# leonsick/depthg

Measured on AMD Instinct MI355X. Metric: correlation-loss steps/sec at B=32,C=384,28x28 (fwd+bwd, per-GPU batch 32), higher is better.
Workload: dtype bf16 (feats) / f16 (code) MFMA inputs, f32 accumulate

## Files before the change

depthg_amd/csrc/dg_api_corr.hip:

```cpp
#include "dg_api.h"
#include "dg_corr_args.h"
#include "dg_taps.h"

static unsigned long long* g_prof_span = nullptr;
extern "C" int dg_prof_main_span(void* span) { g_prof_span = static_cast<unsigned long long*>(span); return DG_OK; }

enum class Prep { Small, Dense, General };
enum class Sampler { Plane, ChannelLast };
enum class MainKernel { Small, Corr2, CorrMain };
enum class Depth { None, Job, GsBlocks, GsOwnLaunch };
enum class Hist { Rows, Blobs };
enum class Masks { None, Sampled, DenseRaw, DenseSplit };

struct PairSet {
    int op;
    int neg;
    bool mapped;
    float shift;
    int slot_loss, slot_cd;
    float fin_scale;
    int gidx, csel, dest;
    float factor;
};
struct Operand {
    int srcsel;
    int cset;
    int map;
};

struct Plan {
    int B, C, D, h, w, hc, wc, S, Sh, P, Ppad, KF, KD, C4, D4, N, T, nops, rf, nrb;
    bool shared, depth, grad, pointwise;
    Prep prep;
    Sampler sampler;
    MainKernel main;
    Masks masks;
    Hist hist;
    bool fold;
    bool half;
    Depth depth_run;
    int nsplit;
    int dep_nrb;
    float lo, hi;
    float shift_depth;
    float inv_numel;
    float grad_f, grad_fn;
    int blob, blob_off_c;
    PairSet ps[DG_MAX_NEG + 2];
    Operand ops[DG_MAX_NEG + 2];
    bool gr_on;
    int gr_nkeys, gr_cpb, gr_blocks_per_image;
    int8_t gr_key[DG_MAX_JOBS], gr_first[DG_MAX_JOBS];
    int32_t gr_nblk[DG_MAX_JOBS];
    size_t nhwc_f[2], nhwc_c[2];
    size_t rows_f[DG_MAX_NEG + 2], rows_c[DG_MAX_NEG + 2];
    size_t op[DG_MAX_NEG + 2], inv[DG_MAX_NEG + 2], colpart[DG_MAX_NEG + 2], bbar[DG_MAX_NEG + 2];
    size_t ccolpart[DG_MAX_NEG + 2], csum[DG_MAX_NEG + 2], bsplit[DG_MAX_NEG + 2];
    size_t rvec[DG_MAX_NEG + 2], rimg[DG_MAX_NEG + 2];
    size_t nz, nzsum;
    size_t dRA[DG_MAX_NEG + 3], dRB[DG_MAX_NEG + 2];
    size_t part[DG_MAX_NEG + 3];
    size_t comb[2], scratch_out, taps, gbuf[DG_MAX_NEG + 2];
    size_t ticket;
    size_t maskbits[DG_MAX_NEG + 2];
    size_t clo[2];
    size_t gr_list, gr_count, gr_rank;
    size_t dRA2[DG_MAX_NEG + 2], dRBs[DG_MAX_NEG + 2], dRB2[DG_MAX_NEG + 2][2], dRBm[DG_MAX_NEG + 2], part4, om;
    size_t total;

    bool small() const { return prep == Prep::Small; }
    bool dense() const { return prep == Prep::Dense; }
    bool plane() const { return sampler == Sampler::Plane; }
    bool has_masks() const { return masks != Masks::None; }
    bool depth_in_gs() const { return depth_run == Depth::GsBlocks || depth_run == Depth::GsOwnLaunch; }
    bool dense_masks() const { return masks == Masks::DenseRaw || masks == Masks::DenseSplit; }
    bool intra_symmetric() const { return !pointwise || fold; }
    const int64_t* batch_map(int k, const int64_t* perms) const {
        return k < 0 ? nullptr : reinterpret_cast<const int64_t*>(reinterpret_cast<uintptr_t>(perms) + (size_t)k * B * sizeof(int64_t));
    }
    const int64_t* map_of(int t, const int64_t* perms) const { return batch_map(ps[t].mapped ? ps[t].neg : -1, perms); }
};

static inline float* f32(char* ws, size_t off) { return reinterpret_cast<float*>(ws + off); }

#define FOLD_STASH_OFF (5 * 1024)

static void plan_tables(const dg_corr_desc* d, Plan& p) {
    const double numel = (double)p.B * p.P * p.P;
    p.inv_numel = (float)(1.0 / numel);
    p.grad_f = (float)(-1.0 / numel);
    p.grad_fn = p.N > 0 ? p.grad_f / (float)p.N : 0.f;
    for (int t = 0; t < p.T; ++t) {
        PairSet& s = p.ps[t];
        const bool neg = t >= 2;
        s.neg = neg ? t - 2 : -1;
        s.mapped = neg && p.shared;
        s.op = s.mapped ? 0 : t;
        s.shift = t == 0 ? d->shift_intra : (t == 1 ? d->shift_inter : d->shift_neg);
        s.slot_loss = neg ? DG_OUT_LOSS_NEG : t;
        s.slot_cd = neg ? DG_OUT_CD_NEG : DG_OUT_CD_INTRA + t;
        s.fin_scale = neg ? (float)(1.0 / (numel * p.N)) : p.inv_numel;
        s.gidx = neg ? 2 : t; s.csel = t == 0 ? 0 : 1; s.dest = t == 1 ? 1 : 0;
        s.factor = neg ? p.grad_fn : p.grad_f;
    }
    for (int o = 0; o < p.nops; ++o) p.ops[o] = Operand{o == 1 ? 1 : 0, o == 0 ? 0 : 1, o >= 2 ? o - 2 : -1};
    const int L = (p.Ppad / 32) % 8;
    if (!(p.grad && p.KF == 384 && p.KD == 96 && p.D <= 80 && p.nrb > 1 && L >= 1 && L <= 4 && p.B % 8 == 0 && p.B <= 64)) return;
    int nkeys = 0, members[DG_MAX_JOBS] = {0};
    for (int t = 0; t < p.T; ++t) {
        int k = -1;
        for (int q = 0; q < nkeys; ++q) if (p.ps[p.gr_first[q]].op == p.ps[t].op) k = q;
        if (k < 0) { k = nkeys++; p.gr_first[k] = (int8_t)t; }
        p.gr_key[t] = (int8_t)k; ++members[k];
    }
    for (int k = 0; k < nkeys; ++k) p.gr_on |= members[k] > 1;
    if (!p.gr_on) return;
    p.gr_nkeys = nkeys; p.gr_cpb = 8 / L;
// ... 66 lines not shown
    for (int i = 0; i < p.nops; ++i) { p.rows_f[i] = take(want_rows ? B * p.P * frow : 0); p.rows_c[i] = take(want_rows ? B * p.P * p.D4 * 4 : 0); }
    for (int i = 0; i < p.nops; ++i) {
        p.op[i] = take(B * (p.Ppad / 32) * (size_t)p.blob);
        p.inv[i] = take(B * p.Ppad * 4);
        p.colpart[i] = take(B * (size_t)(ident ? p.h * ((p.w + 31) / 32) : p.Ppad / 32) * p.KF * 4);
        p.bbar[i] = take(B * p.KF * 4);
        p.bsplit[i] = take(B * 2 * p.KF * 2);
        p.ccolpart[i] = take(B * (size_t)(p.Ppad / 32) * p.KD * 4);
        p.csum[i] = take(B * p.KD * 4);
    }
    for (int t = 0; t < p.T; ++t) { p.rvec[t] = take(B * p.Ppad * 4); p.rimg[t] = take(B * 4); }
    p.nz = take(B * p.Ppad * 4);
    p.nzsum = take(B * 4);
    for (int t = 0; t <= p.T; ++t) { p.dRA[t] = take(B * p.Ppad * p.KD * 4); p.part[t] = take(B * p.nrb * 2 * 4); }
    for (int t = 0; t < p.T; ++t) p.dRB[t] = take(B * p.Ppad * p.KD * 4);
    for (int i = 0; i < 2; ++i) p.comb[i] = take(B * p.Ppad * p.KD * 4);
    p.scratch_out = take(DG_OUT_COUNT * 4);
    p.taps = take(2 * B * dg_taps_record_bytes(p.hc * p.wc, p.P));
    for (int t = 0; t < p.T; ++t) p.gbuf[t] = p.grad ? take(B * (size_t)(p.Ppad / 32) * (p.Ppad / 32) * 2048) : 0;
    p.ticket = take(256);
    const bool xmask = rows && !p.small() && p.grad && plain_zero_clamp && p.Ppad <= 256 && p.rf == 4;
    const bool xmask_dense = (d->flags & DG_EXACT_MASKS) && ident && p.grad && plain_zero_clamp &&
                             p.KF == 384 && p.KD == 96 && p.D <= 80 && p.Ppad >= 160 && p.B <= 64;
    if ((d->flags & DG_EXACT_MASKS) && p.grad && (d->flags & DG_ZERO_CLAMP) && !xmask && !xmask_dense && !p.small())
        return fail(DG_ERR_UNSUPPORTED, "DG_EXACT_MASKS: exact clamp masks exist on small sample grids (always on there) and on the dense "
                                        "identity grid with C <= 384 (padded to 384), D <= 80, P >= 160, B <= 64, zero_clamp without stabalize");
    p.masks = xmask ? Masks::Sampled : (!xmask_dense ? Masks::None : (p.pointwise ? Masks::DenseSplit : Masks::DenseRaw));
    for (int t = 0; t < p.T; ++t) p.maskbits[t] = take(p.has_masks() ? B * (size_t)(p.Ppad / 32) * p.Ppad * 4 : 0);
    p.main = p.small() ? MainKernel::Small
                       : (p.grad && dg_corr2_shape_supported(p.KF, p.KD, p.D, p.lo, p.hi, p.Ppad, p.B) ? MainKernel::Corr2 : MainKernel::CorrMain);
    static const bool fold_on = [] { const char* e = getenv("DG_FOLD_INTRA"); return !(e && e[0] == '0'); }();
    p.fold = fold_on && p.main == MainKernel::Corr2 && p.pointwise && !xmask;
    p.half = p.main == MainKernel::Corr2 && ident && p.N * p.B <= 512 && p.S == p.h && p.S == p.w;
    p.depth_run = (!p.depth || p.small()) ? Depth::None : (!p.grad ? Depth::Job : (p.dense_masks() ? Depth::GsOwnLaunch : Depth::GsBlocks));
    for (int i = 0; i < 2; ++i) p.clo[i] = take(p.masks == Masks::DenseSplit ? B * (size_t)(p.Ppad / 32) * p.KD * 64 : 0);
    p.gr_list = take((size_t)DG_MAX_JOBS * B * DG_GR_CAP * 4);
    p.gr_count = take((size_t)DG_MAX_JOBS * B * 4);
    p.gr_rank = take((size_t)DG_MAX_JOBS * B * 2);
    {
        const bool sg = p.small() && p.grad, two = sg && p.pointwise;
        const size_t gt = B * p.Ppad * p.KD * 4;
        for (int t = 0; t < p.T; ++t) {
            p.dRA2[t] = take(two ? gt : 0);
            p.dRBs[t] = take(sg && p.nsplit == 2 ? gt : 0);
            for (int k = 0; k < 2; ++k) p.dRB2[t][k] = take(two && k < p.nsplit ? gt : 0);
            p.dRBm[t] = take(sg && t >= 2 && (p.pointwise || p.nsplit == 2) ? gt : 0);
        }
        p.part4 = take(p.small() ? (size_t)(p.T + 1) * B * p.nsplit * 16 : 0);
        p.om = take(p.small() ? (size_t)(p.T + 1) * 4 : 0);
    }
    p.total = off;
    plan_tables(d, p);
    return DG_OK;
}

extern "C" size_t dg_corr_workspace_bytes(const dg_corr_desc* desc) {
    Plan p{};
    if (make_plan(desc, p) != DG_OK) return 0;
    return p.total;
}

static DgJob helper_job(const Plan& p, char* ws, int t, bool passB, const int64_t* perms) {
    DgJob j;
    memset(&j, 0, sizeof(j));
    const int o2 = p.ps[t].op;
    const int64_t* m2 = p.map_of(t, perms);
// ... 312 lines not shown
    DgColmeanArgs m;
    memset(&m, 0, sizeof(m));
    m.nops = p.nops; m.B = p.B; m.P = p.P; m.Ppad = p.Ppad; m.KF = p.KF; m.KD = p.KD;
    for (int o = 0; o < p.nops; ++o) {
        m.colpart[o] = p.pointwise ? f32(c.ws, p.colpart[o]) : nullptr; m.bbar[o] = f32(c.ws, p.bbar[o]);
        m.bsplit[o] = reinterpret_cast<__bf16*>(c.ws + p.bsplit[o]);
        m.ngroups[o] = p.Ppad / 32;
        m.ccolpart[o] = f32(c.ws, p.ccolpart[o]); m.csum[o] = f32(c.ws, p.csum[o]);
    }
    m.zero_word = p.depth_in_gs() ? reinterpret_cast<unsigned int*>(c.ws + p.ticket) : nullptr;
    m.zero_words9 = a.wctr;
    if (p.gr_on) {
        m.gr.nh = p.T; m.gr.nkeys = p.gr_nkeys; m.gr.B = p.B;
        for (int t = 0; t < p.T; ++t) { m.gr.sidx[t] = p.map_of(t, c.perms); m.gr.key[t] = p.gr_key[t]; }
        m.gr.list = reinterpret_cast<int32_t*>(c.ws + p.gr_list); m.gr.count = reinterpret_cast<int32_t*>(c.ws + p.gr_count);
        m.gr.rank = reinterpret_cast<int16_t*>(c.ws + p.gr_rank);
    }
    if (p.dense() && p.pointwise) {
        m.dc.code[0] = c.code; m.dc.code[1] = c.code_pos;
        for (int o = 0; o < 2; ++o) { m.dc.blob[o] = c.ws + p.op[o]; m.dc.inv_norm[o] = f32(c.ws, p.inv[o]); m.dc.ccolpart[o] = f32(c.ws, p.ccolpart[o]); }
        m.dc.B = p.B; m.dc.D = p.D; m.dc.KF = p.KF; m.dc.KD = p.KD; m.dc.h = p.h; m.dc.w = p.w; m.dc.P = p.P; m.dc.Ppad = p.Ppad;
        if (p.masks == Masks::DenseSplit) { m.dc.clo[0] = c.ws + p.clo[0]; m.dc.clo[1] = c.ws + p.clo[1]; }
    }
    if (c.split) {
        DgColmeanArgs ms = m;
        ms.zsel = 1; m.zsel = 2;
        DG_HIP(c.side->hand_over(0));
        DG_HIP(dg_launch_colmean(ms, c.side->stream()));
    }
    DG_HIP(dg_launch_colmean(m, c.stream));
    return DG_OK;
}

static int fwd_cd_mask3(Fwd& c) {
    const Plan& p = c.p;
    DgCdMask3Args m;
    memset(&m, 0, sizeof(m));
    m.opR = c.ws + p.op[0]; m.loR = c.ws + p.clo[0];
    for (int t = 0; t < p.T; ++t) {
        m.opS[t] = c.ws + p.op[p.ps[t].op]; m.loS[t] = c.ws + p.clo[p.ps[t].op]; m.sidx[t] = p.map_of(t, c.perms);
        m.bits[t] = reinterpret_cast<uint32_t*>(c.ws + p.maskbits[t]);
    }
    m.T = p.T; m.B = p.B; m.Ppad = p.Ppad; m.blob_bytes = p.blob; m.off_c = p.blob_off_c; m.KD = p.KD;
    if (c.split) {
        DG_HIP(c.side->hand_over(1));
        DG_HIP(dg_launch_cd_mask3(m, c.side->stream()));
        DG_HIP(c.side->record_join());
    } else {
        DG_HIP(dg_launch_cd_mask3(m, c.stream));
    }
    return DG_OK;
}

static int fwd_rowmeans(Fwd& c) {
    const Plan& p = c.p;
    DgRowmeanArgs r;
    memset(&r, 0, sizeof(r));
    r.B = p.B; r.P = p.P; r.Ppad = p.Ppad; r.KF = p.KF; r.KD = p.KD; r.njobs = p.T; r.abar = f32(c.ws, p.bbar[0]);
    for (int t = 0; t < p.T; ++t) {
        r.jobs[t].A = c.ws + p.op[0]; r.jobs[t].aidx = nullptr;
        r.jobs[t].bbar = f32(c.ws, p.bbar[p.ps[t].op]); r.jobs[t].bidx = p.map_of(t, c.perms);
        r.jobs[t].bsplit = reinterpret_cast<const __bf16*>(c.ws + p.bsplit[p.ps[t].op]);
        r.jobs[t].rvec = f32(c.ws, p.rvec[t]); r.jobs[t].rimg = f32(c.ws, p.rimg[t]);
    }
    if (p.dense()) {
        r.ncs = 2;
// ... 51 lines not shown
        DG_HIP(side.fork());
        DG_HIP(dg_launch_gs(g, dep_maskbits, side.stream(), true));
        DG_HIP(side.record_join());
        DG_HIP(dg_launch_gs(gstream, nullptr, c.stream, false, p.half));
        DG_HIP(side.join());
    } else {
        DG_HIP(dg_launch_gs(gstream, nullptr, c.stream, false, p.half));
        DG_HIP(dg_launch_gs(g, dep_maskbits, c.stream, true));
    }
    return DG_OK;
}

static int corr_forward_impl(const dg_corr_desc* desc, const float* orig_feats, const float* orig_feats_pos,
                             const float* orig_code, const float* orig_code_pos, const float* depth,
                             const float* coords1, const float* coords2, const int64_t* perms, const DrawArgs* draw,
                             float* out_scalars, void* workspace, size_t workspace_bytes, dg_stream_t stream_,
                             const FeatKeep* fk = nullptr, const float* feat_inv = nullptr) {
    Fwd c;
    if (int rc = make_plan(desc, c.p)) return rc;
    const Plan& p = c.p;
    c.desc = desc; c.feats = orig_feats; c.feats_pos = orig_feats_pos; c.code = orig_code; c.code_pos = orig_code_pos; c.depth = depth;
    c.coords1 = coords1; c.coords2 = coords2; c.perms = perms; c.draw = draw; c.fk = fk; c.feat_inv = feat_inv; c.out = out_scalars;
    c.stream = static_cast<hipStream_t>(stream_);
    if (int rc = fwd_validate(c, workspace, workspace_bytes)) return rc;

    if (p.dense_masks() && split_masks_enabled()) c.side.emplace(c.stream);
    c.split = c.side && static_cast<bool>(*c.side) && p.pointwise;

    if (p.small()) return forward_small(c);
    if (int rc = p.dense() ? fwd_operands_dense(c) : fwd_operands_general(c)) return rc;

    build_corr_jobs(p, c.ws, perms, c.a);

    if (int rc = fwd_colmeans(c)) return rc;
    if (p.masks == Masks::DenseSplit) { if (int rc = fwd_cd_mask3(c)) return rc; }
    if (p.pointwise) { if (int rc = fwd_rowmeans(c)) return rc; }

    if (c.split) DG_HIP(c.side->join());
    if (int rc = launch_main(p, c.a, c.stream)) return rc;

    return fwd_finish(c);
}

extern "C" int dg_corr_forward(const dg_corr_desc* desc, const float* orig_feats, const float* orig_feats_pos,
                               const float* orig_code, const float* orig_code_pos, const float* depth,
                               const float* coords1, const float* coords2, const int64_t* perms,
                               float* out_scalars, void* workspace, size_t workspace_bytes, dg_stream_t stream_) {
    return corr_forward_impl(desc, orig_feats, orig_feats_pos, orig_code, orig_code_pos, depth, coords1, coords2, perms, nullptr,
                             out_scalars, workspace, workspace_bytes, stream_);
}

extern "C" int dg_corr_forward_extnorm(const dg_corr_desc* desc, const float* orig_feats, const float* orig_feats_pos,
                                       const float* orig_code, const float* orig_code_pos, const float* depth,
                                       const float* coords1, const float* coords2, const int64_t* perms, const float* feat_inv,
                                       float* out_scalars, void* workspace, size_t workspace_bytes, dg_stream_t stream_) {
    if (!feat_inv) return fail(DG_ERR_INVALID, "dg_corr_forward_extnorm: feat_inv is null");
    return corr_forward_impl(desc, orig_feats, orig_feats_pos, orig_code, orig_code_pos, depth, coords1, coords2, perms, nullptr,
                             out_scalars, workspace, workspace_bytes, stream_, nullptr, feat_inv);
}

extern "C" int dg_sampled_sumsq(int32_t B, int32_t C, int32_t h, int32_t w, int32_t S, int32_t line_grid, const float* feats,
                                const float* coords, const int64_t* srcidx, int32_t accumulate, float* out, dg_stream_t stream_) {
    if (B < 1 || C < 1 || h < 1 || w < 1 || S < 1 || !feats || !coords || !out) return fail(DG_ERR_INVALID, "dg_sampled_sumsq: bad arguments");
    DG_HIP(dg_launch_sampled_sumsq(feats, coords, srcidx, out, B, C, h, w, S, line_grid ? 1 : S, accumulate ? 1 : 0, static_cast<hipStream_t>(stream_)));
    return DG_OK;
}

extern "C" int dg_corr_forward_draw(const dg_corr_desc* desc, const float* orig_feats, const float* orig_feats_pos,
                                    const float* orig_code, const float* orig_code_pos, const float* depth,
// ... 238 lines not shown
```

depthg_amd/csrc/dg_corr_args.h:

```cpp
#pragma once
#include "dg_device.h"

__host__ __device__ inline int dg_perm32(int pl) {
    int s = pl >> 4, u = (pl >> 3) & 1, hh = (pl >> 2) & 1, v = pl & 3;
    return (2 * s + hh) * 8 + 4 * u + v;
}

#ifndef DG_F_IG
#define DG_F_IG 4
#endif
__host__ __device__ inline int dg_f_off(int q, int g) {
    constexpr int IG = DG_F_IG;
    return ((g / IG) * 32 + q) * (IG * 16) + (((g % IG) ^ ((q / (16 / IG)) % IG)) * 16);
}

struct DgBlob {
    int GF, GD, KD;
    int off_c, off_p, bytes;
    __host__ __device__ DgBlob(int KF, int KD_) : GF(KF / 8), GD(KD_ / 8), KD(KD_) {
        off_c = 32 * GF * 16;
        off_p = off_c + GD * 32 * 16;
        bytes = off_p + 4 * KD * 16;
    }
    __host__ __device__ int f(int q, int g) const { return dg_f_off(q, g); }
// ... 338 lines not shown
struct DgColmeanArgs {
    const float* colpart[DG_MAX_NEG + 2];
    float* bbar[DG_MAX_NEG + 2];
    __bf16* bsplit[DG_MAX_NEG + 2];
    const float* ccolpart[DG_MAX_NEG + 2];
    float* csum[DG_MAX_NEG + 2];
    int32_t ngroups[DG_MAX_NEG + 2];
    int32_t nops, B, P, Ppad, KF, KD;
    unsigned int* zero_word;
    unsigned int* zero_words9;
    DgGroupArgs gr;
    DgDenseCodeArgs dc;
    int32_t zsel;
};

struct DgRowmeanJob {
    const char* A;
    const float* bbar;
    const __bf16* bsplit;
    const int64_t* aidx;
    const int64_t* bidx;
    float* rvec;
    float* rimg;
};
struct DgRowmeanArgs {
    DgRowmeanJob jobs[DG_MAX_NEG + 2];
    int32_t njobs, B, P, Ppad, KF, KD;
    const float* abar;
    char* stash;
    int32_t stash_off;
    const float* cs_part[2];
    float* cs_out[2];
    int32_t ncs;
};

struct DgScatterSrc {
    const float* buf;
    const int64_t* route;
    int32_t gidx;
    int32_t coords_sel;
    float factor;
    int32_t dest;
    int32_t raw;
    const float* dfac;
    int32_t half;
};
#define DG_MAX_SCATTER 48
struct DgScatterArgs {
    DgScatterSrc src[DG_MAX_SCATTER];
    int32_t nsrc;
    const float* coords1;
    const float* coords2;
    const float* gscal;
    const float* gtot;
    float wtot[4];
    float* comb[2];
    char* taps;
    const char* xop;
    const float* xinv;
    const float* xinv_dest[2];
    int32_t blob_bytes, blob_off_c;
    float* out[2];
    int32_t B, D, DP, h, w, S, Sh, P, Ppad, DC;
    int32_t dense;
    int8_t craw[2][DG_MAX_SCATTER / 2], cfin[2][DG_MAX_SCATTER / 2];
    int8_t ncraw[2], ncfin[2];
// ... 45 lines not shown
hipError_t dg_launch_gs(const struct DgGsArgs& a, const uint32_t* dep_maskbits, hipStream_t s, bool depth_only = false, bool half_out = false);
hipError_t dg_launch_finish(const DgFinishArgs& a, hipStream_t stream);
hipError_t dg_launch_transpose(const DgTransposeArgs& a, int B, hipStream_t s);
hipError_t dg_launch_gather(const DgGatherArgs& a, int maxK, hipStream_t s);
hipError_t dg_launch_cd_mask(const DgCdMaskArgs& a, hipStream_t s);
struct DgCdMask3Args {
    const char* opR;
    const char* loR;
    const char* opS[DG_MAX_NEG + 2];
    const char* loS[DG_MAX_NEG + 2];
    const int64_t* sidx[DG_MAX_NEG + 2];
    uint32_t* bits[DG_MAX_NEG + 2];
    int32_t T, B, Ppad, blob_bytes, off_c, KD;
    int32_t nsplit;
};
hipError_t dg_launch_cd_mask3(const DgCdMask3Args& a, hipStream_t s);
#define DG_HIST_MAX_BINS 256
struct DgCdHistArgs {
    const char* opR;
    const char* opS[DG_MAX_NEG + 2];
    const float* rowsR;
    const float* rowsS[DG_MAX_NEG + 2];
    const int64_t* sidx[DG_MAX_NEG + 2];
    unsigned long long* out;
    int32_t count, B, P, Ppad, D, D4, KD, blob_bytes, off_c;
    int32_t nbins;
    float lo, scale;
};
hipError_t dg_launch_cd_hist(const DgCdHistArgs& a, bool rows, hipStream_t s);
hipError_t dg_launch_plane_sample(const DgPlaneArgs& a, hipStream_t s);
hipError_t dg_launch_colmean(const DgColmeanArgs& a, hipStream_t s);
hipError_t dg_launch_prep_dense(const DgDenseArgs& a, hipStream_t s);
hipError_t dg_launch_rowmean(const DgRowmeanArgs& a, hipStream_t s);
hipError_t dg_launch_set_stash(char* blobs, int B, int ntiles, size_t blob_bytes, int off, const float* rvec, int P, int Ppad, hipStream_t s);
hipError_t dg_launch_scatter(const DgScatterArgs& a, hipStream_t s);
hipError_t dg_launch_super_perms(const float* keys, uint64_t seed, unsigned long long* state, int count, int B, int64_t* out, hipStream_t s);
hipError_t dg_launch_pre_general(const struct DgPreArgs& a, hipStream_t s);
bool dg_small_supported(int Ppad, int KD);
hipError_t dg_launch_corr_small(const struct DgSmallArgs& a, hipStream_t s);
hipError_t dg_launch_small_finish(const struct DgSmallArgs& a, hipStream_t s);
hipError_t dg_launch_gather_rows(const struct DgGatherRowsArgs& a, hipStream_t s);
hipError_t dg_launch_rand_coords_state(unsigned long long* state, float* out, int n, hipStream_t s, float keep_p = -1.f);
hipError_t dg_launch_fps(const float* depth, const float* depth_b, int Ba, int B, int H, int W, int h, int w, int S, float factor,
                         float* out_coords, int32_t* out_inds, float* pooled_ws, hipStream_t s);
hipError_t dg_launch_sampled_sumsq(const float* feats, const float* coords, const int64_t* srcidx, float* out, int B, int C, int h, int w, int S, int Sh, int accumulate, hipStream_t s);
hipError_t dg_launch_normalize_split(const float* src, int B, int C, int P, int nchunks, int chunk_c, float* const* dst, hipStream_t s);
```

depthg_amd/csrc/dg_prep.hip:

```cpp
#include "dg_device.h"
#include "dg_corr_args.h"
#include "dg_taps.h"
#include <cstdlib>

__global__ void k_nchw_to_nhwc(const DgTransposeArgs a) {
    __shared__ float t[32][33];
    const int b = blockIdx.z;
    int m = 0, gy = blockIdx.y;
    while (m < a.nmaps - 1 && gy >= (a.K4[m] + 31) / 32) { gy -= (a.K4[m] + 31) / 32; ++m; }
    const float* __restrict__ src = a.src[m];
    float* __restrict__ dst = a.dst[m];
    const int K = a.K[m], K4 = a.K4[m], HW = a.HW[m];
    const int k0 = gy * 32, p0 = blockIdx.x * 32;
    if (p0 >= HW) return;
    const int tx = threadIdx.x, ty = threadIdx.y;
    for (int i = ty; i < 32; i += 8) {
        int k = k0 + i, p = p0 + tx;
        t[i][tx] = (k < K && p < HW) ? src[((size_t)b * K + k) * HW + p] : 0.f;
    }
    __syncthreads();
    for (int i = ty; i < 32; i += 8) {
        int p = p0 + i, k = k0 + tx;
        if (p < HW && k < K4) dst[((size_t)b * HW + p) * K4 + k] = t[tx][i];
    }
// ... 664 lines not shown
            v[e] = *reinterpret_cast<const _Float16*>(xt + (tl * 32 + pl) * RS + d * 2);
        }
        *reinterpret_cast<f16x8*>(blob0 + (size_t)tl * L.bytes + L.p(d, cc)) = v;
    }
    for (int id = tid; id < ntile * KD; id += 256) {
        const int tl = id / KD, d = id - tl * KD;
        float cs = 0.f;
#pragma unroll 8
        for (int qq = 0; qq < 32; ++qq) cs += (float)*reinterpret_cast<const _Float16*>(xt + (tl * 32 + qq) * RS + d * 2);
        a.ccolpart[o][((size_t)n * nt + t0 + tl) * KD + d] = cs;
    }
}

template <int UN>
__device__ __forceinline__ void prep_dense_code_norms(const DgDenseArgs& a, int xb, int n, int o) {
    const int HW = a.h * a.w, i = xb * 256 + threadIdx.x;
    float* inv = a.inv_norm[o] + (size_t)n * a.Ppad;
    if (xb == 0)
        for (int p = a.P + threadIdx.x; p < a.Ppad; p += 256) inv[p] = 0.f;
    if (i >= HW) return;
    const float* src = a.code[o] + (size_t)n * a.D * HW + i;
    float t[4 * UN];
#pragma unroll
    for (int k = 0; k < 4 * UN; ++k) t[k] = k < a.D ? src[(size_t)k * HW] : 0.f;
    float ss[4] = {0.f, 0.f, 0.f, 0.f};
#pragma unroll
    for (int u = 0; u < UN; ++u)
#pragma unroll
        for (int kg = 0; kg < 4; ++kg) ss[kg] = fmaf(t[kg + 4 * u], t[kg + 4 * u], ss[kg]);
    const float tot = ss[0] + ss[1] + ss[2] + ss[3];
    inv[i] = 1.f / fmaxf(sqrtf(tot), DG_EPS_NORM);
}

__device__ __forceinline__ void dense_code_planes(const DgDenseCodeArgs& a, char* xt, int n, int o, int g) {
    const int tid = threadIdx.x, HW = a.h * a.w, nt = a.Ppad / 32, KD = a.KD;
    const DgBlob L(a.KF, a.KD);
    const int nch = min(8, a.D - 8 * g);
    char* const xl = xt + (size_t)a.Ppad * 16;
    const bool want_lo = a.clo[o] != nullptr;
    for (int p = a.P + tid; p < a.Ppad; p += 256) {
        reinterpret_cast<uint4*>(xt)[p] = make_uint4(0u, 0u, 0u, 0u);
        if (want_lo) reinterpret_cast<uint4*>(xl)[p] = make_uint4(0u, 0u, 0u, 0u);
    }
    if (nch <= 0) {
        for (int p = tid; p < a.P; p += 256) {
            reinterpret_cast<uint4*>(xt)[p] = make_uint4(0u, 0u, 0u, 0u);
            if (want_lo) reinterpret_cast<uint4*>(xl)[p] = make_uint4(0u, 0u, 0u, 0u);
        }
    } else {
        const float* src = a.code[o] + ((size_t)n * a.D + 8 * g) * HW;
        const float* inv = a.inv_norm[o] + (size_t)n * a.Ppad;
        for (int i0 = 0; i0 < HW; i0 += 1024) {
            float t[4][8], iv[4];
            int pp[4];
#pragma unroll
            for (int j = 0; j < 4; ++j) {
                const int i = i0 + tid + 256 * j;
                const bool ok = i < HW;
                pp[j] = ok ? i : -1;
                iv[j] = ok ? inv[pp[j]] : 0.f;
#pragma unroll
                for (int c = 0; c < 8; ++c) t[j][c] = (ok && c < nch) ? src[(size_t)c * HW + i] : 0.f;
            }
#pragma unroll
            for (int j = 0; j < 4; ++j) {
                if (pp[j] < 0) continue;
                f16x8 v;
#pragma unroll
                for (int c = 0; c < 8; ++c) v[c] = c < nch ? (_Float16)(t[j][c] * iv[j]) : (_Float16)0.f;
                *reinterpret_cast<f16x8*>(xt + pp[j] * 16) = v;
                if (want_lo) {
                    f16x8 l;
#pragma unroll
                    for (int c = 0; c < 8; ++c) l[c] = c < nch ? (_Float16)((t[j][c] * iv[j] - (float)v[c]) * 2048.f) : (_Float16)0.f;
                    *reinterpret_cast<f16x8*>(xl + pp[j] * 16) = l;
                }
            }
        }
    }
    __syncthreads();
    char* blob0 = a.blob[o] + (size_t)n * nt * L.bytes;
    for (int id = tid; id < nt * 32; id += 256) {
        const int tl = id >> 5, qq = id & 31;
        *reinterpret_cast<uint4*>(blob0 + (size_t)tl * L.bytes + L.c(qq, g)) = reinterpret_cast<const uint4*>(xt)[id];
        if (want_lo)
            *reinterpret_cast<uint4*>(a.clo[o] + ((size_t)n * nt + tl) * (KD * 64) + (g * 32 + qq) * 16) = reinterpret_cast<const uint4*>(xl)[id];
    }
    for (int id = tid; id < nt * 32; id += 256) {
        const int tl = id >> 5, cc = (id >> 3) & 3, c = id & 7;
        f16x8 v;
#pragma unroll
        for (int e = 0; e < 8; ++e) {
            const int pl = 16 * (cc >> 1) + 8 * ((e >> 2) & 1) + 4 * (cc & 1) + (e & 3);
            v[e] = *reinterpret_cast<const _Float16*>(xt + (tl * 32 + pl) * 16 + c * 2);
        }
        *reinterpret_cast<f16x8*>(blob0 + (size_t)tl * L.bytes + L.p(8 * g + c, cc)) = v;
    }
    for (int id = tid; id < nt * 8; id += 256) {
        const int tl = id >> 3, c = id & 7;
        float cs = 0.f;
#pragma unroll 8
        for (int qq = 0; qq < 32; ++qq) cs += (float)*reinterpret_cast<const _Float16*>(xt + (tl * 32 + qq) * 16 + c * 2);
        a.ccolpart[o][((size_t)n * nt + tl) * KD + 8 * g + c] = cs;
    }
}


template <int MAXU, int UNC, bool FK = false>
__global__ __launch_bounds__(256) void k_prep_dense(const DgDenseArgs a) {
    extern __shared__ float sl[];
    int bid;
    {
        const int nwg = gridDim.x, orig = blockIdx.x;
        const int q = nwg >> 3, rem = nwg & 7, xcd = orig & 7;
        bid = (xcd < rem ? xcd * (q + 1) : rem * (q + 1) + (xcd - rem) * q) + (orig >> 3);
    }
    const int gx = a.Ppad / 32;
    const int nz = a.depth ? 5 : 4;
    const int x = bid % gx, z = (bid / gx) % nz, n = bid / (gx * nz);
    const int roles = a.roles ? a.roles : 15;
    if (n >= a.B) {
        if (roles & 8) dg_super_perm_row(nullptr, a.draw_seed, a.draw_state, a.B, a.draw_out, bid - gx * nz * a.B, a.draw_count, sl);
        return;
    }
    if (!(roles & (z < 2 ? 1 : (z < 4 ? 2 : 4)))) return;
    if (z < 2) {
        prep_dense_feats<MAXU, FK>(a, sl, x, n, z);
    } else if (z < 4) {
        if (a.code_split) {
            if (x * 256 < a.h * a.w) prep_dense_code_norms<UNC>(a, x, n, z - 2);
        } else if (x * DENSE_TPB < a.Ppad / 32) prep_dense_code<UNC>(a, sl, x, n, z - 2);
    } else if (x == 0) {
        depth_nz_image(a.depth, a.nz, a.nzsum, n, a.dH, a.dW, a.h, a.h, a.Ppad, true);
    }
}

// ... 96 lines not shown
__device__ __forceinline__ void colsum_reduce(const float* part, int n, int ngroups, int K, float scale, float* out) {
    for (int k = threadIdx.x; k < K; k += blockDim.x) {
        const float* cp = part + (size_t)n * ngroups * K + k;
        float s = 0.f;
        int t = 0;
        for (; t + 16 <= ngroups; t += 16) {
            float v[16];
#pragma unroll
            for (int u = 0; u < 16; ++u) v[u] = cp[(size_t)(t + u) * K];
#pragma unroll
            for (int u = 0; u < 16; ++u) s += v[u];
        }
        for (; t + 4 <= ngroups; t += 4) {
            float v[4];
#pragma unroll
            for (int u = 0; u < 4; ++u) v[u] = cp[(size_t)(t + u) * K];
#pragma unroll
            for (int u = 0; u < 4; ++u) s += v[u];
        }
        for (; t < ngroups; ++t) s += cp[(size_t)t * K];
        out[(size_t)n * K + k] = s * scale;
    }
}

__global__ __launch_bounds__(256) void k_colmean(const DgColmeanArgs a) {
    extern __shared__ __attribute__((aligned(16))) char cm_smem[];
    const int n = blockIdx.x, o = blockIdx.y;
    if (a.zero_word && n == 0 && o == 0 && blockIdx.z == 0 && threadIdx.x == 0) *a.zero_word = 0u;
    if (a.zero_words9 && n == 0 && o == 0 && blockIdx.z == 0 && threadIdx.x < 9) a.zero_words9[threadIdx.x] = 0u;
    auto reduce = [&](const float* part, int ngroups, int K, float scale, float* out) __attribute__((always_inline)) { colsum_reduce(part, n, ngroups, K, scale, out); };
    if (a.zsel == 1 ? blockIdx.z != 3 : (a.zsel == 2 && blockIdx.z == 3)) return;
    if (blockIdx.z == 3) {
        const int GD = a.dc.KD / 8;
        if ((int)blockIdx.y < 2 * GD) dense_code_planes(a.dc, cm_smem, n, (int)blockIdx.y / GD, (int)blockIdx.y % GD);
        return;
    }
    if (blockIdx.z == 2) {
        if ((int)blockIdx.y < a.gr.nkeys && threadIdx.x < 64) dg_group_lists(a.gr, n, o, threadIdx.x);
        return;
    }
    if (o >= a.nops) return;
    if (blockIdx.z == 0 && a.colpart[o]) {
        reduce(a.colpart[o], a.ngroups[o], a.KF, 1.f / (float)a.P, a.bbar[o]);
        __syncthreads();
        for (int k = threadIdx.x; k < a.KF; k += 256) {
            const float v = a.bbar[o][(size_t)n * a.KF + k];
            const __bf16 hi = (__bf16)v;
            a.bsplit[o][((size_t)n * 2) * a.KF + k] = hi;
            a.bsplit[o][((size_t)n * 2 + 1) * a.KF + k] = (__bf16)(v - (float)hi);
        }
    }
    if (blockIdx.z == 1 && a.ccolpart[o] && a.dc.B == 0) reduce(a.ccolpart[o], a.Ppad / 32, a.KD, 1.f, a.csum[o]);
}

hipError_t dg_launch_colmean(const DgColmeanArgs& a, hipStream_t s) {
    int ny = a.gr.nkeys > a.nops ? a.gr.nkeys : a.nops;
    int nz = a.gr.nkeys > 0 ? 3 : 2, smem = 0;
    if (a.dc.B > 0) {
        if (a.nops != 2) return hipErrorInvalidValue;
        ny = max(ny, 2 * (a.dc.KD / 8)); nz = 4; smem = a.dc.Ppad * 16 * ((a.dc.clo[0] || a.dc.clo[1]) ? 2 : 1);
        hipError_t e = dg_set_max_smem(reinterpret_cast<const void*>(k_colmean), smem);
        if (e != hipSuccess) return e;
    }
    hipLaunchKernelGGL(k_colmean, dim3(a.B, ny, nz), dim3(256), smem, s, a);
    return hipGetLastError();
}

// ... 73 lines not shown
        if (has && !lo) J.rvec[(size_t)n * a.Ppad + p] = p < a.P ? v : 0.f;
        if (a.stash && has && !lo && jb == 0) {
            const float x = p < a.P ? -0.5f * v : 0.f;
            const _Float16 xh = (_Float16)x, xl = (_Float16)((x - (float)xh) * 2048.f);
            const uint32_t word = (uint32_t)__builtin_bit_cast(unsigned short, xh) | ((uint32_t)__builtin_bit_cast(unsigned short, xl) << 16);
            *reinterpret_cast<uint32_t*>(a.stash + ((size_t)n * nt + tile) * L.bytes + L.off_c + a.stash_off + (p & 31) * 16) = word;
        }
    }
}
__global__ __launch_bounds__(64) void k_set_stash(char* blobs, size_t blob_bytes, int off, const float* rvec, int ntiles, int P, int Ppad) {
    if (threadIdx.x >= 32) return;
    uint32_t word = 0u;
    if (rvec) {
        const int n = (int)blockIdx.x / ntiles, tile = (int)blockIdx.x - n * ntiles, p = tile * 32 + (int)threadIdx.x;
        const float x = p < P ? -0.5f * rvec[(size_t)n * Ppad + p] : 0.f;
        const _Float16 xh = (_Float16)x, xl = (_Float16)((x - (float)xh) * 2048.f);
        word = (uint32_t)__builtin_bit_cast(unsigned short, xh) | ((uint32_t)__builtin_bit_cast(unsigned short, xl) << 16);
    }
    *reinterpret_cast<uint32_t*>(blobs + (size_t)blockIdx.x * blob_bytes + off + threadIdx.x * 16) = word;
}
hipError_t dg_launch_set_stash(char* blobs, int B, int ntiles, size_t blob_bytes, int off, const float* rvec, int P, int Ppad, hipStream_t s) {
    hipLaunchKernelGGL(k_set_stash, dim3(B * ntiles), dim3(64), 0, s, blobs, blob_bytes, off, rvec, ntiles, P, Ppad);
    return hipGetLastError();
}

hipError_t dg_launch_rowmean(const DgRowmeanArgs& a, hipStream_t s) {
    if (a.njobs > 16) return hipErrorInvalidValue;
    const int smem = max(32 * (a.KF / 8) * 16, (ROWMEAN_WAVES - 1) * 16 * 64 * 4);
    hipError_t e = dg_set_max_smem(reinterpret_cast<const void*>(k_rowmean), smem);
    if (e != hipSuccess) return e;
    hipLaunchKernelGGL(k_rowmean, dim3(a.Ppad / 32 + 1 + (a.ncs > 0 ? 1 : 0), a.B), dim3(64 * ROWMEAN_WAVES), smem, s, a);
    return hipGetLastError();
}
```

Measured before the change: 3272.

## Fuse dense column means, row means, code planes and group lists into one kernel

On the dense pointwise path without masks, the colmean, code-plane and rowmean launches are replaced by a single 1024-thread kernel. Its blocks split into three roles: column-mean reduction followed by MFMA row-mean products and the fold stash, code-plane transposition with csum computed in place, and group-list building. This removes at least one launch and the separate reduction round trips between the stages. In exchange the kernel is large, needs a lot of LDS, and its row-mean blocks each redo the column reduction, so that work is repeated per tile group.

After: 3297, median of 6. No clear change (+0.8%).

```diff
diff --git a/depthg_amd/csrc/dg_api_corr.hip b/depthg_amd/csrc/dg_api_corr.hip
--- a/depthg_amd/csrc/dg_api_corr.hip
+++ b/depthg_amd/csrc/dg_api_corr.hip
@@ -39,6 +39,7 @@
     bool fold;
     bool half;
     Depth depth_run;
+    bool dense_means;
     int nsplit;
     int dep_nrb;
     float lo, hi;
@@ -83,6 +84,7 @@
 
 static inline float* f32(char* ws, size_t off) { return reinterpret_cast<float*>(ws + off); }
 
+#define DENSE_MEANS_MAX_TILES 128
 #define FOLD_STASH_OFF (5 * 1024)
 
 static void plan_tables(const dg_corr_desc* d, Plan& p) {
@@ -215,6 +217,7 @@
     static const bool fold_on = [] { const char* e = getenv("DG_FOLD_INTRA"); return !(e && e[0] == '0'); }();
     p.fold = fold_on && p.main == MainKernel::Corr2 && p.pointwise && !xmask;
     p.half = p.main == MainKernel::Corr2 && ident && p.N * p.B <= 512 && p.S == p.h && p.S == p.w;
+    p.dense_means = p.dense() && p.pointwise && p.masks == Masks::None && p.Ppad / 32 <= DENSE_MEANS_MAX_TILES;
     p.depth_run = (!p.depth || p.small()) ? Depth::None : (!p.grad ? Depth::Job : (p.dense_masks() ? Depth::GsOwnLaunch : Depth::GsBlocks));
     for (int i = 0; i < 2; ++i) p.clo[i] = take(p.masks == Masks::DenseSplit ? B * (size_t)(p.Ppad / 32) * p.KD * 64 : 0);
     p.gr_list = take((size_t)DG_MAX_JOBS * B * DG_GR_CAP * 4);
@@ -593,6 +596,34 @@
     return DG_OK;
 }
 
+static int fwd_dense_means(Fwd& c) {
+    const Plan& p = c.p;
+    DgDenseMeansArgs m;
+    memset(&m, 0, sizeof(m));
+    m.njobs = p.T; m.B = p.B; m.P = p.P; m.Ppad = p.Ppad; m.KF = p.KF; m.KD = p.KD;
+    m.A = c.ws + p.op[0];
+    for (int t = 0; t < p.T; ++t) {
+        m.jobs[t].colpart = f32(c.ws, p.colpart[p.ps[t].op]); m.jobs[t].bidx = p.map_of(t, c.perms);
+        m.jobs[t].rvec = f32(c.ws, p.rvec[t]); m.jobs[t].rimg = f32(c.ws, p.rimg[t]);
+    }
+    for (int o = 0; o < 2; ++o) {
+        m.bbar[o] = f32(c.ws, p.bbar[o]); m.bsplit[o] = reinterpret_cast<__bf16*>(c.ws + p.bsplit[o]); m.csum[o] = f32(c.ws, p.csum[o]);
+        m.dc.code[o] = o ? c.code_pos : c.code; m.dc.blob[o] = c.ws + p.op[o]; m.dc.inv_norm[o] = f32(c.ws, p.inv[o]); m.dc.ccolpart[o] = f32(c.ws, p.ccolpart[o]);
+    }
+    m.dc.B = p.B; m.dc.D = p.D; m.dc.KF = p.KF; m.dc.KD = p.KD; m.dc.h = p.h; m.dc.w = p.w; m.dc.P = p.P; m.dc.Ppad = p.Ppad;
+    if (p.fold) { m.stash = c.ws + p.op[0]; m.stash_off = FOLD_STASH_OFF; }
+    m.zero_word = p.depth_in_gs() ? reinterpret_cast<unsigned int*>(c.ws + p.ticket) : nullptr;
+    m.zero_words9 = c.a.wctr;
+    if (p.gr_on) {
+        m.gr.nh = p.T; m.gr.nkeys = p.gr_nkeys; m.gr.B = p.B;
+        for (int t = 0; t < p.T; ++t) { m.gr.sidx[t] = p.map_of(t, c.perms); m.gr.key[t] = p.gr_key[t]; }
+        m.gr.list = reinterpret_cast<int32_t*>(c.ws + p.gr_list); m.gr.count = reinterpret_cast<int32_t*>(c.ws + p.gr_count);
+        m.gr.rank = reinterpret_cast<int16_t*>(c.ws + p.gr_rank);
+    }
+    DG_HIP(dg_launch_dense_means(m, c.stream));
+    return DG_OK;
+}
+
 static int fwd_cd_mask3(Fwd& c) {
     const Plan& p = c.p;
     DgCdMask3Args m;
@@ -710,9 +741,13 @@
 
     build_corr_jobs(p, c.ws, perms, c.a);
 
-    if (int rc = fwd_colmeans(c)) return rc;
-    if (p.masks == Masks::DenseSplit) { if (int rc = fwd_cd_mask3(c)) return rc; }
-    if (p.pointwise) { if (int rc = fwd_rowmeans(c)) return rc; }
+    if (p.dense_means) {
+        if (int rc = fwd_dense_means(c)) return rc;
+    } else {
+        if (int rc = fwd_colmeans(c)) return rc;
+        if (p.masks == Masks::DenseSplit) { if (int rc = fwd_cd_mask3(c)) return rc; }
+        if (p.pointwise) { if (int rc = fwd_rowmeans(c)) return rc; }
+    }
 
     if (c.split) DG_HIP(c.side->join());
     if (int rc = launch_main(p, c.a, c.stream)) return rc;
diff --git a/depthg_amd/csrc/dg_corr_args.h b/depthg_amd/csrc/dg_corr_args.h
--- a/depthg_amd/csrc/dg_corr_args.h
+++ b/depthg_amd/csrc/dg_corr_args.h
@@ -394,6 +394,29 @@
     const float* cs_part[2];
     float* cs_out[2];
     int32_t ncs;
+};
+
+#define DG_DENSE_MEANS_J 4
+struct DgDenseMeansJob {
+    const float* colpart;
+    const int64_t* bidx;
+    float* rvec;
+    float* rimg;
+};
+struct DgDenseMeansArgs {
+    DgDenseMeansJob jobs[DG_MAX_NEG + 2];
+    int32_t njobs, B, P, Ppad, KF, KD;
+    const char* A;
+    float* bbar[2];
+    __bf16* bsplit[2];
+    float* csum[2];
+    char* stash;
+    int32_t stash_off;
+    unsigned int* zero_word;
+    unsigned int* zero_words9;
+    DgGroupArgs gr;
+    DgDenseCodeArgs dc;
+    int32_t pj;
 };
 
 struct DgScatterSrc {
@@ -505,6 +528,7 @@
 hipError_t dg_launch_colmean(const DgColmeanArgs& a, hipStream_t s);
 hipError_t dg_launch_prep_dense(const DgDenseArgs& a, hipStream_t s);
 hipError_t dg_launch_rowmean(const DgRowmeanArgs& a, hipStream_t s);
+hipError_t dg_launch_dense_means(const DgDenseMeansArgs& a, hipStream_t s);
 hipError_t dg_launch_set_stash(char* blobs, int B, int ntiles, size_t blob_bytes, int off, const float* rvec, int P, int Ppad, hipStream_t s);
 hipError_t dg_launch_scatter(const DgScatterArgs& a, hipStream_t s);
 hipError_t dg_launch_super_perms(const float* keys, uint64_t seed, unsigned long long* state, int count, int B, int64_t* out, hipStream_t s);
diff --git a/depthg_amd/csrc/dg_prep.hip b/depthg_amd/csrc/dg_prep.hip
--- a/depthg_amd/csrc/dg_prep.hip
+++ b/depthg_amd/csrc/dg_prep.hip
@@ -720,17 +720,20 @@
     inv[i] = 1.f / fmaxf(sqrtf(tot), DG_EPS_NORM);
 }
 
-__device__ __forceinline__ void dense_code_planes(const DgDenseCodeArgs& a, char* xt, int n, int o, int g) {
-    const int tid = threadIdx.x, HW = a.h * a.w, nt = a.Ppad / 32, KD = a.KD;
+__device__ __forceinline__ void dense_code_planes(const DgDenseCodeArgs& a, char* xt, int n, int o, int g, const int tid,
+                                                  const bool act = true, const int keep_g = -1, float* csum = nullptr) {
+    const int HW = a.h * a.w, nt = a.Ppad / 32, KD = a.KD;
     const DgBlob L(a.KF, a.KD);
     const int nch = min(8, a.D - 8 * g);
     char* const xl = xt + (size_t)a.Ppad * 16;
     const bool want_lo = a.clo[o] != nullptr;
-    for (int p = a.P + tid; p < a.Ppad; p += 256) {
+    float* const cst = reinterpret_cast<float*>(xt + (size_t)a.Ppad * 16 * (want_lo ? 2 : 1));
+    for (int p = a.P + tid; act && p < a.Ppad; p += 256) {
         reinterpret_cast<uint4*>(xt)[p] = make_uint4(0u, 0u, 0u, 0u);
         if (want_lo) reinterpret_cast<uint4*>(xl)[p] = make_uint4(0u, 0u, 0u, 0u);
     }
-    if (nch <= 0) {
+    if (!act) {
+    } else if (nch <= 0) {
         for (int p = tid; p < a.P; p += 256) {
             reinterpret_cast<uint4*>(xt)[p] = make_uint4(0u, 0u, 0u, 0u);
             if (want_lo) reinterpret_cast<uint4*>(xl)[p] = make_uint4(0u, 0u, 0u, 0u);
@@ -768,13 +771,21 @@
     }
     __syncthreads();
     char* blob0 = a.blob[o] + (size_t)n * nt * L.bytes;
-    for (int id = tid; id < nt * 32; id += 256) {
+    const bool keep = o == 0 && g == keep_g;
+    for (int id = tid; act && id < nt * 32; id += 256) {
         const int tl = id >> 5, qq = id & 31;
-        *reinterpret_cast<uint4*>(blob0 + (size_t)tl * L.bytes + L.c(qq, g)) = reinterpret_cast<const uint4*>(xt)[id];
+        const uint4 v = reinterpret_cast<const uint4*>(xt)[id];
+        char* const dst = blob0 + (size_t)tl * L.bytes + L.c(qq, g);
+        if (keep) {
+            *reinterpret_cast<uint32_t*>(dst + 4) = v.y;
+            *reinterpret_cast<uint2*>(dst + 8) = make_uint2(v.z, v.w);
+        } else {
+            *reinterpret_cast<uint4*>(dst) = v;
+        }
         if (want_lo)
             *reinterpret_cast<uint4*>(a.clo[o] + ((size_t)n * nt + tl) * (KD * 64) + (g * 32 + qq) * 16) = reinterpret_cast<const uint4*>(xl)[id];
     }
-    for (int id = tid; id < nt * 32; id += 256) {
+    for (int id = tid; act && id < nt * 32; id += 256) {
         const int tl = id >> 5, cc = (id >> 3) & 3, c = id & 7;
         f16x8 v;
 #pragma unroll
@@ -784,12 +795,20 @@
         }
         *reinterpret_cast<f16x8*>(blob0 + (size_t)tl * L.bytes + L.p(8 * g + c, cc)) = v;
     }
-    for (int id = tid; id < nt * 8; id += 256) {
+    for (int id = tid; act && id < nt * 8; id += 256) {
         const int tl = id >> 3, c = id & 7;
         float cs = 0.f;
 #pragma unroll 8
         for (int qq = 0; qq < 32; ++qq) cs += (float)*reinterpret_cast<const _Float16*>(xt + (tl * 32 + qq) * 16 + c * 2);
         a.ccolpart[o][((size_t)n * nt + tl) * KD + 8 * g + c] = cs;
+        if (csum) cst[id] = cs;
+    }
+    if (!csum) return;
+    __syncthreads();
+    if (act && tid < 8) {
+        float s = 0.f;
+        for (int tl = 0; tl < nt; ++tl) s += cst[tl * 8 + tid];
+        csum[(size_t)n * KD + 8 * g + tid] = s;
     }
 }
 
@@ -952,7 +971,7 @@
     if (a.zsel == 1 ? blockIdx.z != 3 : (a.zsel == 2 && blockIdx.z == 3)) return;
     if (blockIdx.z == 3) {
         const int GD = a.dc.KD / 8;
-        if ((int)blockIdx.y < 2 * GD) dense_code_planes(a.dc, cm_smem, n, (int)blockIdx.y / GD, (int)blockIdx.y % GD);
+        if ((int)blockIdx.y < 2 * GD) dense_code_planes(a.dc, cm_smem, n, (int)blockIdx.y / GD, (int)blockIdx.y % GD, threadIdx.x);
         return;
     }
     if (blockIdx.z == 2) {
@@ -1092,3 +1111,178 @@
     hipLaunchKernelGGL(k_rowmean, dim3(a.Ppad / 32 + 1 + (a.ncs > 0 ? 1 : 0), a.B), dim3(64 * ROWMEAN_WAVES), smem, s, a);
     return hipGetLastError();
 }
+
+#define DENSE_MEANS_THREADS 1024
+__device__ __forceinline__ void lds_only_barrier() { asm volatile("s_waitcnt lgkmcnt(0)\n\ts_barrier" ::: "memory"); }
+
+template <int NKS>
+__device__ __forceinline__ void dense_means_block(const DgDenseMeansArgs& a, char* sm, const int n, const int j) {
+    const int tid = threadIdx.x, lane = tid & 63, c = lane & 31, h = lane >> 5;
+    const int wv = __builtin_amdgcn_readfirstlane(tid >> 6), grp = wv >> 2, wid = wv & 3;
+    constexpr int KF = NKS * 64;
+    const int nt = a.Ppad / 32, T = a.njobs;
+    const int per = (nt + DG_DENSE_MEANS_J - 1) / DG_DENSE_MEANS_J, t0 = j * per, t1 = min(nt, t0 + per);
+    if (t0 >= t1) return;
+    const DgBlob L(KF, a.KD);
+    constexpr int RSB = KF * 2 + 16;
+    float* const mean = reinterpret_cast<float*>(sm);
+    char* const split = sm + (size_t)T * KF * 4;
+    float* const red = reinterpret_cast<float*>(split + (size_t)T * 2 * RSB) + grp * (3 * 16 * 64);
+    const char* const A0 = a.A + (size_t)n * nt * L.bytes;
+    constexpr int AB = NKS > 6 ? 6 : NKS;
+    bf16x8 af[AB];
+    static_assert(DG_F_IG == 4 && NKS % 2 == 0 && AB % 2 == 0, "the k-steps of a wave start at a group of four granules");
+    const uint32_t lp[2] = {(uint32_t)dg_f_off(c, h), (uint32_t)dg_f_off(c, 2 + h)};
+    auto load_a = [&](int tile, int part) __attribute__((always_inline)) {
+        const char* fp = A0 + (size_t)min(tile, t1 - 1) * L.bytes + (wid * NKS + part * AB) * 1024;
+#pragma unroll
+        for (int i = 0; i < AB; ++i) af[i] = *reinterpret_cast<const bf16x8*>(fp + (i >> 1) * 2048 + lp[i & 1]);
+    };
+    constexpr bool A_EARLY = NKS <= 6;
+    if constexpr (A_EARLY) load_a(t0 + grp, 0);
+    const float scale = 1.f / (float)a.P;
+    for (int cg = wv; cg < T * NKS; cg += DENSE_MEANS_THREADS / 64) {
+        const int t = cg / NKS, k = (cg - t * NKS) * 64 + lane;
+        const DgDenseMeansJob& J = a.jobs[t];
+        const int nb = J.bidx ? (int)J.bidx[n] : n;
+        const float* cp = J.colpart + (size_t)nb * nt * KF;
+        float s = 0.f;
+        for (int tb = 0; tb < nt; tb += 32) {
+            float v[32];
+#pragma unroll
+            for (int u = 0; u < 32; ++u) v[u] = (cp + (size_t)min(tb + u, nt - 1) * KF)[k];
+#pragma unroll
+            for (int u = 0; u < 32; ++u) s += tb + u < nt ? v[u] : 0.f;
+        }
+        const float m = dg_mul_rn(s, scale);
+        const __bf16 hi = (__bf16)m, lo = (__bf16)(m - (float)hi);
+        mean[t * KF + k] = m;
+        *reinterpret_cast<__bf16*>(split + (size_t)(2 * t) * RSB + k * 2) = hi;
+        *reinterpret_cast<__bf16*>(split + (size_t)(2 * t + 1) * RSB + k * 2) = lo;
+        if (j == 0 && t < 2) {
+            a.bbar[t][(size_t)n * KF + k] = m;
+            a.bsplit[t][((size_t)n * 2) * KF + k] = hi;
+            a.bsplit[t][((size_t)n * 2 + 1) * KF + k] = lo;
+        }
+    }
+    if constexpr (!A_EARLY) load_a(t0 + grp, 0);
+    lds_only_barrier();
+    if (j == 0) {
+        float av[12];
+#pragma unroll
+        for (int q = 0; q < 12; ++q) av[q] = lane + 64 * q < KF ? mean[lane + 64 * q] : 0.f;
+        for (int t = wv; t < T; t += DENSE_MEANS_THREADS / 64) {
+            const float* bt = mean + t * KF;
+            float s = 0.f;
+#pragma unroll
+            for (int q = 0; q < 12; ++q) s = fmaf(av[q], lane + 64 * q < KF ? bt[lane + 64 * q] : 0.f, s);
+#pragma unroll
+            for (int o = 32; o > 0; o >>= 1) s += __shfl_xor(s, o, 64);
+            if (lane == 0) a.jobs[t].rimg[n] = s * (float)a.P;
+        }
+    }
+    const int jb = c & 15, lo = c >> 4;
+    const bool has = jb < T;
+    const char* const bb = split + (size_t)((has ? jb : 0) * 2 + lo) * RSB + 16 * h;
+    float* const rv = a.jobs[has ? jb : 0].rvec + (size_t)n * a.Ppad;
+    for (int tb = t0; tb < t1; tb += 4) {
+        const int tile = tb + grp;
+        const bool act = tile < t1;
+        f32x16 acc = {};
+#pragma unroll
+        for (int part = 0; part < NKS / AB; ++part) {
+            if (part > 0) load_a(tile, part);
+#pragma unroll
+            for (int i = 0; i < AB; ++i) {
+                bf16x8 b = *reinterpret_cast<const bf16x8*>(bb + 32 * (wid * NKS + part * AB + i));
+                if (!has) {
+#pragma unroll
+                    for (int e = 0; e < 8; ++e) b[e] = (__bf16)0.f;
+                }
+                acc = __builtin_amdgcn_mfma_f32_32x32x16_bf16(af[i], b, acc, 0, 0, 0);
+            }
+        }
+        if (tb + 4 < t1) load_a(tile + 4, 0);
+        lds_only_barrier();
+        if (wid > 0) {
+#pragma unroll
+            for (int i = 0; i < 16; ++i) red[((wid - 1) * 16 + i) * 64 + lane] = acc[i];
+        }
+        lds_only_barrier();
+        if (wid != 0 || !act) continue;
+#pragma unroll
+        for (int w = 0; w < 3; ++w)
+#pragma unroll
+            for (int i = 0; i < 16; ++i) acc[i] += red[(w * 16 + i) * 64 + lane];
+        const int p0 = tile * 32 + 4 * h;
+        float* const rvp = rv + p0;
+        char* const sp = a.stash + ((size_t)n * nt + tile) * L.bytes + L.off_c + a.stash_off + 64 * h;
+        const bool stash = a.stash && has && !lo && jb == 0;
+#pragma unroll
+        for (int i = 0; i < 16; ++i) {
+            const float v = acc[i] + __shfl(acc[i], (lane + 16) & 63, 64);
+            const int r = (i & 3) + 8 * (i >> 2), p = p0 + r;
+            if (has && !lo) rvp[r] = p < a.P ? v : 0.f;
+            if (stash) {
+                const float x = p < a.P ? -0.5f * v : 0.f;
+                const _Float16 xh = (_Float16)x, xl = (_Float16)((x - (float)xh) * 2048.f);
+                const uint32_t word = (uint32_t)__builtin_bit_cast(unsigned short, xh) | ((uint32_t)__builtin_bit_cast(unsigned short, xl) << 16);
+                *reinterpret_cast<uint32_t*>(sp + r * 16) = word;
+            }
+        }
+    }
+}
+
+template <int NKS>
+__global__ __launch_bounds__(DENSE_MEANS_THREADS) void k_dense_means(const DgDenseMeansArgs a) {
+    extern __shared__ __attribute__((aligned(16))) char dm_smem[];
+    const int bid = blockIdx.x, tid = threadIdx.x;
+    if (bid == 0) {
+        if (a.zero_word && tid == 0) *a.zero_word = 0u;
+        if (a.zero_words9 && tid < 9) a.zero_words9[tid] = 0u;
+    }
+    const int nmeans = a.B * DG_DENSE_MEANS_J;
+    if (bid < nmeans) {
+        dense_means_block<NKS>(a, dm_smem, bid % a.B, bid / a.B);
+        return;
+    }
+    const int GD = a.KD / 8, njobs = a.B * 2 * GD, nplane = (njobs + 2 * a.pj - 1) / (2 * a.pj);
+    if (bid < nmeans + nplane) {
+        const int q = __builtin_amdgcn_readfirstlane(tid >> 8);
+        const size_t qbytes = (size_t)a.Ppad * 16 + (size_t)(a.Ppad / 32) * 32;
+        for (int r = 0; r < 2; ++r) {
+            const int job = ((bid - nmeans) * 2 + r) * a.pj + q;
+            const bool act = q < a.pj && job < njobs;
+            const int jc = act ? job : 0, g = jc % GD, no = jc / GD, o = no & 1;
+            if (r) __syncthreads();
+            dense_code_planes(a.dc, dm_smem + (act ? q : 0) * qbytes, no >> 1, o, g, tid & 255, act, a.stash ? a.stash_off / 512 : -1, a.csum[o]);
+        }
+        return;
+    }
+    const int id = (bid - nmeans - nplane) * (DENSE_MEANS_THREADS / 64) + (tid >> 6);
+    if (id < a.gr.nkeys * a.B) dg_group_lists(a.gr, id % a.B, id / a.B, tid & 63);
+}
+
+hipError_t dg_launch_dense_means(const DgDenseMeansArgs& a_in, hipStream_t s) {
+    DgDenseMeansArgs a = a_in;
+    const int nt = a.Ppad / 32, T = a.njobs;
+    if (T < 2 || T > 16 || a.B < 1 || nt < 1 || a.dc.B != a.B || a.dc.clo[0] || a.dc.clo[1]) return hipErrorInvalidValue;
+    if (a.KF != 128 && a.KF != 384 && a.KF != 768) return hipErrorInvalidValue;
+    constexpr int lds_max = 160 * 1024;
+    const int qbytes = a.Ppad * 16 + nt * 32;
+    a.pj = min(4, lds_max / qbytes);
+    if (a.pj < 1) return hipErrorInvalidValue;
+    const int means_bytes = T * a.KF * 4 + T * 2 * (a.KF * 2 + 16) + 4 * 3 * 16 * 64 * 4;
+    if (means_bytes > lds_max) return hipErrorInvalidValue;
+    const int smem = max(means_bytes, a.pj * qbytes);
+    const int GD = a.KD / 8, nplane = (a.B * 2 * GD + 2 * a.pj - 1) / (2 * a.pj);
+    const int nlist = (a.gr.nkeys * a.B + DENSE_MEANS_THREADS / 64 - 1) / (DENSE_MEANS_THREADS / 64);
+    const dim3 grid(a.B * DG_DENSE_MEANS_J + nplane + nlist);
+    auto launch = [&](auto kern) -> hipError_t {
+        const hipError_t e = dg_set_max_smem(reinterpret_cast<const void*>(kern), smem);
+        if (e != hipSuccess) return e;
+        hipLaunchKernelGGL(kern, grid, dim3(DENSE_MEANS_THREADS), smem, s, a);
+        return hipGetLastError();
+    };
+    return a.KF == 128 ? launch(k_dense_means<2>) : (a.KF == 384 ? launch(k_dense_means<6>) : launch(k_dense_means<12>));
+}
```
